# zgojcic/3D_multiview_reg

Measured on AMD Instinct MI355X. Metric: point-cloud pairs/s (feat+match+filter+SVD), 3DMatch 20k-pt, 1/2/4/8 GPU, higher is better.
Workload: dtype f32 (bf16x3 MFMA operands); 1 GPU; one synthetic 3DMatch-scale scene per GPU (configs[2]): 30 fragments x ~20393 voxels (0.025 m) -> FCGF -> rand 5000 samples -> soft feature-NN for all 435 pairs -> OANet (128ch, 500 clusters, 2 blocks) -> weighted Procrustes -> all-gather of (R,t,conf); sampler=rand, fragments_per_gpu=30, pairs_per_gpu=435, samples=5000, voxels_mean=20393, math=f32eq, oanet_point_layout=chunk-major, spconv_presplit_planes=False, spatial_map_order=False, library=353b56b98378a74a, parallelism=dp1 (one scene per rank, RCCL all-gather of records)

## Files before the change

### 3d_multiview_reg_amd/csrc/oan_attn.hip

```cpp
#include <algorithm>
#include <functional>
#include <vector>

#include "common.hpp"
#include "gemm.hpp"
#include "knobs.hpp"
#include "mfma_bf16.hpp"
#include "prof.hpp"
#include "mvreg.h"

namespace mvr {

using namespace bx;

constexpr int AC = 128;
constexpr int AKB = 32;
constexpr int AQ = 256;
constexpr int ATHREADS = 512;
constexpr int ATL = AQ + 4;
constexpr int PLANE = AC * AKB * 2;
constexpr int IMG = 3 * PLANE;
constexpr int STAGE_B = 2 * IMG;
constexpr int MAX_CLUSTERS = 1024;
constexpr int WROW = 272;
constexpr int WPLANE = 32 * WROW;
constexpr int WIMG = 27 * 1024;
constexpr int USTAGE = WIMG + IMG;
static_assert(3 * WPLANE <= WIMG, "W image padding");
constexpr float LOG2E = 1.4426950408889634f;
constexpr float A_NEG = -3.0e38f;
static_assert(64 * ATL * 4 <= 2 * STAGE_B, "epilogue half tile must fit the stage ring");


__device__ int g_attn_reruns;
constexpr float F16_FLOOR = 0.125f;
constexpr float W_SUM_MAX = 128.f;
__device__ __forceinline__ bool v_row_bad(float rmax) { return !(rmax < F16_RANGE) || (rmax > 0.f && rmax < F16_FLOOR); }

#define SCHED_FENCE() __builtin_amdgcn_sched_barrier(0)

#ifndef ATTN_TRACE
#define ATTN_TRACE 0
#endif
#if ATTN_TRACE
__device__ unsigned long long g_attn_trace[16];
#define ATSTAMP(slot)                                                  \
  do {                                                                 \
    unsigned long long t_;                                             \
    __builtin_amdgcn_sched_barrier(0);                                 \
    asm volatile("s_memtime %0\n\ts_waitcnt lgkmcnt(0)" : "=s"(t_));  \
    __builtin_amdgcn_sched_barrier(0);                                 \
    tr_[prev_] += t_ - tlast_;                                         \
    tlast_ = t_;                                                       \
    prev_ = (slot);                                                    \
  } while (0)
#define ATSTART() unsigned long long tr_[8] = {0, 0, 0, 0, 0, 0, 0, 0}, tlast_ = __builtin_amdgcn_s_memtime(); int prev_ = 7
#define ATEND(base)                                                                  \
  do {                                                                               \
    ATSTAMP(7);                                                                      \
    if ((threadIdx.x & 63) == 0)                                                     \
      for (int q_ = 0; q_ < 8; ++q_) atomicAdd(&g_attn_trace[(base) + q_], tr_[q_]); \
  } while (0)
#else
#define ATSTAMP(slot) do {} while (0)
#define ATSTART() do {} while (0)
#define ATEND(base) do {} while (0)
#endif
#define ATTN_INTERLEAVE6()                          \
  do {                                              \
    _Pragma("unroll") for (int u_ = 0; u_ < 6; ++u_) { \
      __builtin_amdgcn_sched_group_barrier(0x008, 1, 0); \
      __builtin_amdgcn_sched_group_barrier(0x002, 5, 0); \
      __builtin_amdgcn_sched_group_barrier(0x200, 1, 0); \
    }                                               \
  } while (0)
#define ATTN_INTERLEAVE3()                          \
  do {                                              \
    _Pragma("unroll") for (int u_ = 0; u_ < 3; ++u_) { \
      __builtin_amdgcn_sched_group_barrier(0x008, 1, 0); \
      __builtin_amdgcn_sched_group_barrier(0x002, 7, 0); \
      __builtin_amdgcn_sched_group_barrier(0x200, 1, 0); \
    }                                               \
  } while (0)

__device__ __forceinline__ int kord_off(int row, int q) {
  const int s = q >> 2, a = (q >> 1) & 1, h = q & 1;
  return row * 64 + 16 * ((2 * s + h) ^ ((row >> 2) & 3)) + 8 * a;
}
__device__ __forceinline__ Frag kord_frag(const char* img, int row, int s, int h) {
  const int off = row * 64 + 16 * ((2 * s + h) ^ ((row >> 2) & 3));
  Frag f;
  f.h = *reinterpret_cast<const bf16x8*>(img + off);
  f.m = *reinterpret_cast<const bf16x8*>(img + PLANE + off);
  f.l = *reinterpret_cast<const bf16x8*>(img + 2 * PLANE + off);
  return f;
}

template <int X>
__device__ __forceinline__ float swz_x(float v) {
  return __int_as_float(__builtin_amdgcn_ds_swizzle(__float_as_int(v), 0x1F | (X << 10)));
}
__device__ __forceinline__ float half_sum(float v) {
  v += swz_x<1>(v);
  v += swz_x<2>(v);
  v += swz_x<4>(v);
  v += swz_x<8>(v);
  v += swz_x<16>(v);
  return v;
}

__device__ __forceinline__ void pair_block(int nblk, int& p, int& blk) {
  const int b = blockIdx.x, x = b & 7, t = b >> 3;
  blk = t % nblk;
  p = (t / nblk) * 8 + x;
}

constexpr float RESCALE = 8.f;
template <int PSH = 0>
__device__ __forceinline__ void online_softmax(float (&v)[16], float& m, float& l, floatx16 (&O)[4]) {
  float bm = __builtin_fmaxf(__builtin_fmaxf(v[0], v[1]), v[2]);
#pragma unroll
  for (int r = 3; r < 15; r += 2) bm = __builtin_fmaxf(__builtin_fmaxf(bm, v[r]), v[r + 1]);
  bm = fmaxf(bm, v[15]);
  bm = fmaxf(bm, __shfl_xor(bm, 32, 64));
  if (__any(bm > m + RESCALE)) {
    const float mn = fmaxf(m, bm);
    const float alpha = __builtin_amdgcn_exp2f(m - mn);
    m = mn;
    l *= alpha;
#pragma unroll
    for (int cb = 0; cb < 4; ++cb) O[cb] *= alpha;
  }
  const float ms = m - (float)PSH;
  float ps = 0.f;
#pragma unroll
  for (int r = 0; r < 16; ++r) {
    v[r] = __builtin_amdgcn_exp2f(v[r] - ms);
    ps += v[r];
  }
  l += ps;
}

__device__ __forceinline__ int64_t cm_off(int n, int64_t cs) { return (int64_t)(n >> 5) * cs + (n & 31); }

__device__ __forceinline__ void tile_out(float* T, const floatx16 (&O)[4], float inv, bool colok, float* out,
                                         int64_t ld, int64_t cs, int col0, int L, float2* st, int64_t st_tile) {
  const int tid = threadIdx.x, lane = tid & 63, w = tid >> 6, l32 = lane & 31, h = lane >> 5;
  const int col = 32 * w + l32;
  const int Lp = (L + 3) & ~3;
  const int nv = min(max(L - col0 - 128 * h, 0), 128);
  const float rnv = nv > 0 ? 1.f / (float)nv : 0.f;
  bool ok[4];
#pragma unroll
  for (int u = 0; u < 4; ++u) ok[u] = 4 * l32 + u < nv;
// ... 444 lines not shown
  const float* sc; const float* sh; int64_t sps;
  const char* wimg;
  const float* bias;
  const float2* bs;
  const char* dimg;
  int P, N, Kc, nkb, nqb;
  float* out; int64_t ops, old, ocs;
  float2* stats; int64_t st_ld; int st_off;
  int* range;
  const int* guard;
};


__global__ __launch_bounds__(ATHREADS) void oan_unpool_kernel(UnpoolArgs a) {
  __shared__ __attribute__((aligned(16))) char smem[USTAGE + 64 * 1024];
  __shared__ __attribute__((aligned(16))) float bsh[MAX_CLUSTERS];
  __shared__ float2 ssh[AC];
  const int tid = threadIdx.x, lane = tid & 63, w = tid >> 6, l32 = lane & 31, h = lane >> 5;
  int p, nb;
  pair_block(a.nqb, p, nb);
  if (p >= a.P) return;
  const int N = a.N, nkb = a.nkb;
  const char* dimg = a.dimg + (int64_t)p * nkb * IMG;

  auto issue = [&](int kb, int st) {
    char* dst = smem + st * USTAGE;
    for (int off = w * 1024; off < USTAGE; off += 8 * 1024) {
      const char* src = off < WIMG ? a.wimg + (int64_t)kb * WIMG + off : dimg + (int64_t)kb * IMG + (off - WIMG);
      glds16b(src + 16 * lane, dst + off);
    }
  };
  issue(0, 0);

  for (int i = tid; i < nkb * AKB; i += ATHREADS)
    bsh[i] = i < a.Kc ? (a.bias ? a.bias[i] * LOG2E : 0.f) : -__builtin_inff();
  if (tid < AC) ssh[tid] = make_float2(a.sc[(int64_t)p * a.sps + tid], a.sh[(int64_t)p * a.sps + tid]);

  const int n = nb * AQ + 32 * w + l32;
  const bool nok = n < N;
  const int nlast = ((N + 3) & ~3) - 4;
  const float* xb = a.X + (int64_t)p * a.xps + cm_off(min(nb * AQ + 4 * lane, nlast), a.xcs);
  auto qdma = [&](int qt) {
    char* dst = smem + USTAGE + (qt & 1) * 32768;
#pragma unroll
    for (int i = 0; i < 4; ++i) {
      const int r = 4 * w + i;
      glds16b(reinterpret_cast<const char*>(xb + (int64_t)(32 * qt + r) * a.xld), dst + r * 1024);
    }
  };
  qdma(0);
  Frag q[8];
#pragma unroll
  for (int qt = 0; qt < 4; ++qt) {
    if (qt < 3) {
      qdma(qt + 1);
      asm volatile("s_waitcnt vmcnt(4)" ::: "memory");
    } else {
      asm volatile("s_waitcnt vmcnt(0)" ::: "memory");
    }
    __syncthreads();
    const float* xt = reinterpret_cast<const float*>(smem + USTAGE + (qt & 1) * 32768) + 32 * w + l32;
#pragma unroll
    for (int kk = 0; kk < 2; ++kk) {
      const int ks = 2 * qt + kk;
      float v[8];
#pragma unroll
      for (int i = 0; i < 8; ++i) {
        const int c = 16 * ks + 8 * h + i;
        const float2 f = ssh[c];
        const float x = fmaxf(fmaf(xt[(c - 32 * qt) * 256], f.x, f.y), 0.f);
        v[i] = nok ? x : 0.f;
      }
      split8(v, q[ks].h, q[ks].m, q[ks].l);
    }
    __syncthreads();
  }

  floatx16 O[4];
#pragma unroll
  for (int cb = 0; cb < 4; ++cb)
#pragma unroll
    for (int r = 0; r < 16; ++r) O[cb][r] = 0.f;
  float m = A_NEG, l = 0.f;

  const int wbase = l32 * WROW + 16 * h;
  auto read_w = [&](const char* Wi, int ks) {
    const int off = wbase + 32 * ks;
    Frag f;
    f.h = *reinterpret_cast<const bf16x8*>(Wi + off);
    f.m = *reinterpret_cast<const bf16x8*>(Wi + WPLANE + off);
    f.l = *reinterpret_cast<const bf16x8*>(Wi + 2 * WPLANE + off);
    return f;
  };

  asm volatile("s_waitcnt vmcnt(0)" ::: "memory");
  __syncthreads();
  for (int kb = 0; kb < nkb; ++kb) {
    const int st = kb & 1;
    if (kb + 1 < nkb) issue(kb + 1, st ^ 1);
    const char* Wi = smem + st * USTAGE;
    const char* D = Wi + WIMG;
    floatx16 S;
#pragma unroll
    for (int r4 = 0; r4 < 4; ++r4) {
      const float4 b = *reinterpret_cast<const float4*>(bsh + kb * AKB + 8 * r4 + 4 * h);
      S[4 * r4 + 0] = b.x;
      S[4 * r4 + 1] = b.y;
      S[4 * r4 + 2] = b.z;
      S[4 * r4 + 3] = b.w;
    }
    Frag cur = read_w(Wi, 0);
#pragma unroll
    for (int ks = 0; ks < 8; ++ks) {
      Frag nxt;
      if (ks < 7) nxt = read_w(Wi, ks + 1);
      SCHED_FENCE();
      S = mfma6(cur, q[ks], S);
      SCHED_FENCE();
      if (ks < 7) cur = nxt;
    }
    Frag df = kord_frag(D, l32, 0, h);
    float v[16];
#pragma unroll
    for (int r = 0; r < 16; ++r) v[r] = S[r];
    online_softmax(v, m, l, O);
    Frag pf[2];
    split8(v, pf[0].h, pf[0].m, pf[0].l);
    split8(v + 8, pf[1].h, pf[1].m, pf[1].l);
#pragma unroll
    for (int i = 0; i < 8; ++i) {
      const int s = i >> 2, cb = i & 3;
      Frag nxt;
      if (i < 7) nxt = kord_frag(D, 32 * ((i + 1) & 3) + l32, (i + 1) >> 2, h);
      SCHED_FENCE();
      O[cb] = mfma6(df, pf[s], O[cb]);
      SCHED_FENCE();
      if (i < 7) df = nxt;
    }
    asm volatile("s_waitcnt vmcnt(0)" ::: "memory");
    __syncthreads();
  }
  const float lt = l + __shfl_xor(l, 32, 64);
  const float inv = lt > 0.f ? 1.f / lt : 0.f;
  const int ntile = (N + 127) / 128;
  tile_out(reinterpret_cast<float*>(smem), O, inv, nok, a.out + (int64_t)p * a.ops, a.old, a.ocs, nb * AQ, N,
           a.stats ? a.stats + ((int64_t)p * ntile + 2 * nb) * a.st_ld + a.st_off : nullptr, a.st_ld);
}

constexpr int U4T = 256;
constexpr int U4Q = 128;
constexpr int U4QB = 32 * U4Q * 4;
constexpr int U4TL = U4Q + 4;
template <int H> constexpr int u4_wimg() { return planes<H>() * WPLANE; }
template <int H> constexpr int u4_lds() { return 2 * u4_wimg<H>() + ximg_bytes<H>(); }
static_assert(u4_wimg<0>() + 2 * U4QB <= u4_lds<0>() && u4_wimg<1>() + 2 * U4QB <= u4_lds<1>(),
              "prologue quarters (at the second W buffer) fit");
static_assert(64 * U4TL * 4 <= u4_lds<1>(), "epilogue half tile fits");

template <int H>
__global__ __launch_bounds__(U4T, 2) void oan_unpool4_kernel(UnpoolArgs a) {
  constexpr int WI4 = u4_wimg<H>();
  constexpr int XDO = 2 * WI4;
  constexpr int XIMG = ximg_bytes<H>();
  constexpr int WSTR = wimg_stride<H>();
  __shared__ __attribute__((aligned(16))) char smem[u4_lds<H>()];
  __shared__ __attribute__((aligned(16))) float bsh[512];
  __shared__ __attribute__((aligned(16))) float ish[H ? 512 : 4];
  __shared__ float2 ssh[AC];
  if (a.guard) {
    if (*a.guard == 0) return;
    if (blockIdx.x == 0 && threadIdx.x == 0) atomicAdd(&g_attn_reruns, 1);
  }
  const int tid = threadIdx.x, lane = tid & 63, w = tid >> 6, l32 = lane & 31, h = lane >> 5;
  int p, nb;
  pair_block(a.nqb, p, nb);
  if (p >= a.P) return;
  ATSTART();
  ATSTAMP(0);
  const int N = a.N, nkb = a.nkb;
  const char* dimg = a.dimg + (int64_t)p * nkb * XIMG;

  const uint32_t smem_lds = lds_addr(smem);
  const int wu = __builtin_amdgcn_readfirstlane(w);
  auto issue_w = [&](int kb) {
    const uint32_t dst = smem_lds + (uint32_t)((kb & 1) * WI4);
    const char* src = a.wimg + (int64_t)kb * WSTR;
#pragma unroll
    for (int i = 0; i < (WI4 + 4095) / 4096; ++i) {
      const int off = wu * 1024 + 4096 * i;
      if (off < WI4 && off + 16 * lane < WI4) glds16s(src, (uint32_t)(off + 16 * lane), dst + (uint32_t)off);
    }
  };
  auto issue_xd = [&](int kb) {
    const char* src = dimg + (int64_t)kb * XIMG;
#pragma unroll
    for (int i = 0; i < (XIMG + 4095) / 4096; ++i) {
      const int off = wu * 1024 + 4096 * i;
      if (off < XIMG) glds16s(src, (uint32_t)(off + 16 * lane), smem_lds + (uint32_t)(XDO + off));
    }
  };
  issue_w(0);

  for (int i = tid; i < nkb * AKB; i += U4T) {
    const float2 b = a.bs[i];
    bsh[i] = b.x;
    if (H) ish[i] = b.y;
  }
  if (tid < AC) ssh[tid] = make_float2(a.sc[(int64_t)p * a.sps + tid], a.sh[(int64_t)p * a.sps + tid]);

  const int n = nb * U4Q + 32 * w + l32;
  const bool nok = n < N;
  const int nlast = ((N + 3) & ~3) - 4;
  const float* xb = a.X + (int64_t)p * a.xps + cm_off(min(nb * U4Q + 4 * l32, nlast), a.xcs);
  auto qdma = [&](int qt) {
    char* dst = smem + WI4 + (qt & 1) * U4QB;
#pragma unroll
    for (int i = 0; i < 4; ++i) {
      const int r2 = 4 * w + i;
      glds16b(reinterpret_cast<const char*>(xb + (int64_t)(32 * qt + 2 * r2 + h) * a.xld), dst + r2 * 1024);
    }
  };
  qdma(0);
  FragT<H> q[8];
  float xmax = 0.f;
#pragma unroll
  for (int qt = 0; qt < 4; ++qt) {
    if (qt < 3) {
      qdma(qt + 1);
      asm volatile("s_waitcnt vmcnt(4)" ::: "memory");
    } else {
      asm volatile("s_waitcnt vmcnt(0)" ::: "memory");
    }
    __syncthreads();
    const float* xt = reinterpret_cast<const float*>(smem + WI4 + (qt & 1) * U4QB) + 32 * w + l32;
#pragma unroll
    for (int kk = 0; kk < 2; ++kk) {
      const int ks = 2 * qt + kk;
      float v[8];
#pragma unroll
      for (int i = 0; i < 8; ++i) {
        const int c = 16 * ks + 8 * h + i;
        const float2 f = ssh[c];
        const float x = fmaxf(fmaf(xt[(c - 32 * qt) * U4Q], f.x, f.y), 0.f);
        v[i] = nok ? x : 0.f;
        if (H) xmax = fmaxf(xmax, v[i]);
      }
      q[ks] = split8t<H>(v);
    }
    __syncthreads();
  }
  if (H && __any(!(xmax < F16_RANGE)) && lane == 0) atomicOr(a.range, 1);
  issue_xd(0);

  floatx16 O[4];
#pragma unroll
  for (int cb = 0; cb < 4; ++cb)
#pragma unroll
    for (int r = 0; r < 16; ++r) O[cb][r] = 0.f;
  float m = A_NEG, l = 0.f;

  const int wbase = l32 * WROW + 16 * h;
  auto read_w = [&](const char* Wi, int ks) { return ld_frag<H>(Wi + wbase + 32 * ks, WPLANE); };
  auto d_frag = [&](const char* D, int row, int s) {
    return ld_frag<H>(D + row * 64 + 16 * ((2 * s + h) ^ ((row >> 2) & 3)), PLANE);
  };

  for (int kb = 0; kb < nkb; ++kb) {
    ATSTAMP(1);
    if (kb + 1 < nkb) issue_w(kb + 1);
    const char* Wi = smem + (kb & 1) * WI4;
    const char* D = smem + XDO;
    floatx16 S;
#pragma unroll
    for (int r4 = 0; r4 < 4; ++r4) {
      const float4 b = *reinterpret_cast<const float4*>(bsh + kb * AKB + 8 * r4 + 4 * h);
      S[4 * r4 + 0] = b.x;
      S[4 * r4 + 1] = b.y;
      S[4 * r4 + 2] = b.z;
      S[4 * r4 + 3] = b.w;
    }
    FragT<H> cur = read_w(Wi, 0);
#pragma unroll
    for (int ks = 0; ks < 8; ++ks) {
      FragT<H> nxt;
      if (ks < 7) nxt = read_w(Wi, ks + 1);
      SCHED_FENCE();
      S = mma<H>(cur, q[ks], S);
      SCHED_FENCE();
      if (ks < 7) cur = nxt;
    }
    ATSTAMP(2);
    float v[16];
    if (H) {
#pragma unroll
      for (int r4 = 0; r4 < 4; ++r4) {
        const float4 is = *reinterpret_cast<const float4*>(ish + kb * AKB + 8 * r4 + 4 * h);
        v[4 * r4 + 0] = S[4 * r4 + 0] * is.x;
        v[4 * r4 + 1] = S[4 * r4 + 1] * is.y;
        v[4 * r4 + 2] = S[4 * r4 + 2] * is.z;
        v[4 * r4 + 3] = S[4 * r4 + 3] * is.w;
      }
    } else {
#pragma unroll
      for (int r = 0; r < 16; ++r) v[r] = S[r];
    }
    online_softmax<H ? 7 : 0>(v, m, l, O);
    FragT<H> pf[2] = {split8t<H>(v), split8t<H>(v + 8)};
    ATSTAMP(3);
    asm volatile("s_waitcnt vmcnt(0)" ::: "memory");
    __syncthreads();
    ATSTAMP(4);
    FragT<H> df = d_frag(D, l32, 0);
#pragma unroll
    for (int i = 0; i < 8; ++i) {
      const int s = i >> 2, cb = i & 3;
      FragT<H> nxt;
      if (i < 7) nxt = d_frag(D, 32 * ((i + 1) & 3) + l32, (i + 1) >> 2);
      SCHED_FENCE();
      O[cb] = mma<H>(df, pf[s], O[cb]);
      SCHED_FENCE();
      if (i < 7) df = nxt;
    }
    ATSTAMP(5);
    __syncthreads();
    if (kb + 1 < nkb) issue_xd(kb + 1);
  }
  asm volatile("s_waitcnt vmcnt(0)" ::: "memory");
  __syncthreads();
  ATSTAMP(6);

  const float lt = l + __shfl_xor(l, 32, 64);
  const float inv = lt > 0.f ? 1.f / lt : 0.f;
  float* T = reinterpret_cast<float*>(smem);
  const int col0 = nb * U4Q;
  const int nv = min(max(N - col0, 0), U4Q);
  const float rnv = nv > 0 ? 1.f / (float)nv : 0.f;
  bool ok[4];
#pragma unroll
  for (int u = 0; u < 4; ++u) ok[u] = 4 * l32 + u < nv;
  const int Lp = (N + 3) & ~3;
  const bool sok = col0 + 4 * l32 < Lp;
  float* out = a.out + (int64_t)p * a.ops;
  float2* st = a.stats ? a.stats + ((int64_t)p * ((N + 127) / 128) + nb) * a.st_ld + a.st_off : nullptr;
#pragma unroll
  for (int hf = 0; hf < 2; ++hf) {
#pragma unroll
    for (int cc = 0; cc < 2; ++cc)
#pragma unroll
      for (int q2 = 0; q2 < 16; ++q2) {
        const int c = 32 * cc + (q2 & 3) + 8 * (q2 >> 2) + 4 * h;
        T[c * U4TL + 32 * w + l32] = nok ? O[2 * hf + cc][q2] * inv : 0.f;
      }
    __syncthreads();
    for (int it = 0; it < 8; ++it) {
      const int cl = 16 * w + 2 * it + h, c = 64 * hf + cl;
      float4 x = *reinterpret_cast<const float4*>(T + cl * U4TL + 4 * l32);
      if (!ok[0]) x.x = 0.f;
      if (!ok[1]) x.y = 0.f;
      if (!ok[2]) x.z = 0.f;
      if (!ok[3]) x.w = 0.f;
      if (st) {
        const float sm = half_sum((x.x + x.y) + (x.z + x.w));
        const float mu = sm * rnv;
        const float d0 = ok[0] ? x.x - mu : 0.f, d1 = ok[1] ? x.y - mu : 0.f, d2 = ok[2] ? x.z - mu : 0.f,
                    d3 = ok[3] ? x.w - mu : 0.f;
        const float m2 = half_sum((d0 * d0 + d1 * d1) + (d2 * d2 + d3 * d3));
        if (l32 == 0 && nv > 0) st[c] = make_float2(sm, m2);
      }
      if (sok) *reinterpret_cast<float4*>(out + (int64_t)c * a.old + cm_off(col0 + 4 * l32, a.ocs)) = x;
    }
    __syncthreads();
  }
  ATEND(8);
}

#ifndef ATTN_MATH_DEFAULT
#define ATTN_MATH_DEFAULT 0
#endif
int g_attn_h = ATTN_MATH_DEFAULT;

}

using namespace mvr;

static bool al16(const void* p) { return (reinterpret_cast<uintptr_t>(p) & 15) == 0; }
static int64_t round_up4(int64_t x) { return (x + 3) & ~(int64_t)3; }

#if ATTN_TRACE
extern "C" int mvr_attn_trace(unsigned long long* out, int reset) {
  if (hipMemcpyFromSymbol(out, HIP_SYMBOL(mvr::g_attn_trace), sizeof(unsigned long long) * 16) != hipSuccess) return -1;
  if (reset) {
    unsigned long long z[16] = {};
    if (hipMemcpyToSymbol(HIP_SYMBOL(mvr::g_attn_trace), z, sizeof(z)) != hipSuccess) return -1;
  }
  return 0;
}
#endif

extern "C" size_t mvr_oan_diff_unpool_workspace_bytes(int P, int channels, int clusters) {
  if (P <= 0 || channels != AC || clusters <= 0 || clusters > MAX_CLUSTERS) return 0;
  const size_t nkb = (size_t)(clusters + AKB - 1) / AKB;
  return nkb * (WIMG + (size_t)P * IMG + AKB * sizeof(float2)) + 512;
}

struct PoolSplit { int nks, g0; };
#ifndef POOL_TAIL
#define POOL_TAIL 0
#endif
static double pool_makespan(int64_t full, int64_t parts, int k, int cus) {
  std::vector<double> slot((size_t)cus, 0.0);
  std::make_heap(slot.begin(), slot.end(), std::greater<double>());
  auto put = [&](double d) {
    std::pop_heap(slot.begin(), slot.end(), std::greater<double>());
    slot.back() += d;
    std::push_heap(slot.begin(), slot.end(), std::greater<double>());
  };
  for (int64_t i = 0; i < full; ++i) put(1.0);
  for (int64_t i = 0; i < parts; ++i) put(1.0 / k);
  return *std::max_element(slot.begin(), slot.end());
}
static PoolSplit pool_splits(int P, int nqb, int N) {
  const int nkb = (N + AKB - 1) / AKB;
  if (!POOL_TAIL) return nkb >= 16 ? PoolSplit{2, 0} : PoolSplit{1, (P + 7) / 8};
  int dev = 0, cus = 0;
  if (hipGetDevice(&dev) != hipSuccess ||
      hipDeviceGetAttribute(&cus, hipDeviceAttributeMultiprocessorCount, dev) != hipSuccess || cus <= 0)
    cus = 256;
  const int G = (P + 7) / 8;
  const int64_t per = 8LL * nqb;
  PoolSplit best{1, G};
  double tbest = pool_makespan(per * G, 0, 1, cus);
  int64_t slabs_best = 0;
  for (int k = 2; k <= 4; k *= 2) {
    if (nkb < 8 * k) break;
    const int gfill = (int)(((per * G) / cus) * cus / per);
    const int cands[3] = {0, gfill, G};
    for (int g0 : cands) {
      if (g0 >= G) continue;
      const int64_t parts = per * k * (G - g0);
      const double t = pool_makespan(per * g0, parts, k, cus);
      if (t < tbest - 1e-9 || (t < tbest + 1e-9 && parts < slabs_best)) {
        tbest = t;
        best = PoolSplit{k, g0};
        slabs_best = parts;
      }
    }
  }
  return best;
}

static size_t pool_ws_bytes(int P, int clusters, int nks) {
  const size_t slots = (size_t)P * ((clusters + AQ - 1) / AQ);
  return (nks > 1 ? slots * ((size_t)nks * PSLAB * 4 + 4) : 0) + 512;
}


extern "C" size_t mvr_oan_diff_pool_workspace_bytes(int P, int channels, int clusters) {
  if (P <= 0 || channels != AC || clusters <= 0 || clusters > MAX_CLUSTERS) return 0;
  return pool_ws_bytes(P, clusters, 4);
}

extern "C" int mvr_oan_diff_pool_ws(const float* x, int64_t x_pstride, int64_t x_ld, const float* sc,
                                    const float* sh, int64_t s_pstride, const float* weight, const float* bias, int P,
                                    int channels, int N, int clusters, float* out, int64_t out_pstride, int64_t out_ld,
                                    float* stats, int64_t st_ld, int st_off, void* workspace, size_t workspace_bytes,
                                    hipStream_t stream);

extern "C" int mvr_oan_diff_pool(const float* x, int64_t x_pstride, int64_t x_ld, const float* sc, const float* sh,
                                 int64_t s_pstride, const float* weight, const float* bias, int P, int channels, int N,
                                 int clusters, float* out, int64_t out_pstride, int64_t out_ld, float* stats,
                                 int64_t st_ld, int st_off, hipStream_t stream) {
  return mvr_oan_diff_pool_ws(x, x_pstride, x_ld, sc, sh, s_pstride, weight, bias, P, channels, N, clusters, out,
                              out_pstride, out_ld, stats, st_ld, st_off, nullptr, 0, stream);
}

extern "C" int mvr_oan_diff_pool_ws(const float* x, int64_t x_pstride, int64_t x_ld, const float* sc,
                                    const float* sh, int64_t s_pstride, const float* weight, const float* bias, int P,
                                    int channels, int N, int clusters, float* out, int64_t out_pstride, int64_t out_ld,
                                    float* stats, int64_t st_ld, int st_off, void* workspace, size_t workspace_bytes,
                                    hipStream_t stream) {
  return mvr::oan_diff_pool_cm(x, x_pstride, x_ld, 32, sc, sh, s_pstride, weight, bias, P, channels, N, clusters, out,
                               out_pstride, out_ld, stats, st_ld, st_off, workspace, workspace_bytes, stream);
}

int mvr::oan_diff_pool_cm(const float* x, int64_t x_pstride, int64_t x_ld, int64_t x_cs, const float* sc,
                          const float* sh, int64_t s_pstride, const float* weight, const float* bias, int P,
                          int channels, int N, int clusters, float* out, int64_t out_pstride, int64_t out_ld,
                          float* stats, int64_t st_ld, int st_off, void* workspace, size_t workspace_bytes,
                          hipStream_t stream) {
  if (P < 0 || N <= 0 || channels != AC || clusters <= 0 || clusters > MAX_CLUSTERS) return MVR_EINVAL;
  if (P == 0) return MVR_OK;
  if (!x || !sc || !sh || !weight || !out) return MVR_EINVAL;
  const bool xcm = x_cs != 32;
  if ((xcm ? (x_ld != 32 || (x_cs & 3) || x_cs < 32 * AC) : x_ld < round_up4(N)) || (x_ld & 3) || (x_pstride & 3) ||
      !al16(x) || !al16(weight) || !al16(out) || out_ld < round_up4(clusters) || (out_ld & 3) || (out_pstride & 3) ||
      (stats && (st_ld < channels + st_off)))
    return MVR_EINVAL;
  if ((xcm ? (int64_t)((N + 31) / 32) * x_cs : (int64_t)AC * x_ld) * 4 >= ((int64_t)1 << 31)) return MVR_EINVAL;
  if (P == 0) return MVR_OK;
  PoolArgs a{};
  a.X = x; a.xps = x_pstride; a.xld = x_ld; a.xcs = x_cs;
  a.sc = sc; a.sh = sh; a.sps = s_pstride;
  a.W = weight; a.bias = bias;
  a.P = P; a.N = N; a.Kc = clusters; a.nqb = (clusters + AQ - 1) / AQ;
  a.out = out; a.ops = out_pstride; a.old = out_ld;
  a.stats = reinterpret_cast<float2*>(stats); a.st_ld = st_ld; a.st_off = st_off;
  a.nks = 1;
  const size_t slots = (size_t)P * a.nqb;
  int* range = nullptr;
  if (workspace) {
    if (!al16(workspace) || workspace_bytes < pool_ws_bytes(P, clusters, 4)) return MVR_EINVAL;
    const PoolSplit ps = pool_splits(P, a.nqb, N);
    const int k = ps.nks;
    if (k > 1) {
      a.nks = k;
      a.g0 = ps.g0;
      a.part = reinterpret_cast<float*>(workspace);
      a.cnt = reinterpret_cast<int*>(reinterpret_cast<char*>(workspace) + slots * (size_t)k * PSLAB * 4);
    }
    if (g_attn_h)
      range = reinterpret_cast<int*>(reinterpret_cast<char*>(workspace) +
                                     (a.nks > 1 ? slots * ((size_t)a.nks * PSLAB * 4 + 4) : 0));
  }
  if (a.nks > 1 || range) {
    void* z = a.nks > 1 ? (void*)a.cnt : (void*)range;
// ... 116 lines not shown
```

Baseline: 11090 pairs/s.

## Software-pipeline unpool attention: overlap softmax/split with next block's MFMA

Restructures the OANet unpool attention kernel so that the softmax and bf16/f16 operand split for key block j run interleaved with the score MFMAs of block j+1. It also interleaves the output MFMAs, using sched_group_barrier hints and per-plane fragment reloads. The LDS layout changes from a double-buffered W image to a single W image plus double-buffered x_down images, and the prologue gets a deeper ring of X quarter loads. Waves whose columns are entirely out of range now skip the math. The goal is to hide VALU softmax latency behind MFMA and cut serialization, at the cost of more complex scheduling, extra register pressure and a different barrier pattern.

```diff
diff --git a/3d_multiview_reg_amd/csrc/oan_attn.hip b/3d_multiview_reg_amd/csrc/oan_attn.hip
--- a/3d_multiview_reg_amd/csrc/oan_attn.hip
+++ b/3d_multiview_reg_amd/csrc/oan_attn.hip
@@ -1,5 +1,6 @@
 #include <algorithm>
 #include <functional>
+#include <type_traits>
 #include <vector>
 
 #include "common.hpp"
@@ -750,15 +751,62 @@
 constexpr int U4QB = 32 * U4Q * 4;
 constexpr int U4TL = U4Q + 4;
 template <int H> constexpr int u4_wimg() { return planes<H>() * WPLANE; }
-template <int H> constexpr int u4_lds() { return 2 * u4_wimg<H>() + ximg_bytes<H>(); }
+template <int H> constexpr int u4_lds() { return u4_wimg<H>() + 2 * ximg_bytes<H>(); }
 static_assert(u4_wimg<0>() + 2 * U4QB <= u4_lds<0>() && u4_wimg<1>() + 2 * U4QB <= u4_lds<1>(),
-              "prologue quarters (at the second W buffer) fit");
+              "prologue quarters (behind the W image, over the x_down slots) fit");
 static_assert(64 * U4TL * 4 <= u4_lds<1>(), "epilogue half tile fits");
+static_assert(u4_lds<0>() <= 76800, "two workgroups per CU");
+
+template <typename V16>
+__device__ __forceinline__ void softmax_decide(const V16& v, float& m, float& l, float& alpha, bool& resc) {
+  float bm = __builtin_fmaxf(__builtin_fmaxf(v[0], v[1]), v[2]);
+#pragma unroll
+  for (int r = 3; r < 15; r += 2) bm = __builtin_fmaxf(__builtin_fmaxf(bm, v[r]), v[r + 1]);
+  bm = fmaxf(bm, v[15]);
+  bm = fmaxf(bm, __shfl_xor(bm, 32, 64));
+  resc = __any(bm > m + RESCALE);
+  const float mn = fmaxf(m, bm);
+  alpha = __builtin_amdgcn_exp2f(m - mn);
+  l = resc ? l * alpha : l;
+  m = resc ? mn : m;
+}
+template <int H, typename LD>
+__device__ __forceinline__ floatx16 mma_reload(FragT<H>& a, const FragT<H>& b, floatx16 acc, LD ld) {
+  if constexpr (H) {
+    acc = __builtin_amdgcn_mfma_f32_32x32x16_f16(a.p[1], b.p[0], acc, 0, 0, 0);
+    a.p[1] = ld(1);
+    acc = __builtin_amdgcn_mfma_f32_32x32x16_f16(a.p[0], b.p[1], acc, 0, 0, 0);
+    acc = __builtin_amdgcn_mfma_f32_32x32x16_f16(a.p[0], b.p[0], acc, 0, 0, 0);
+  } else {
+    acc = __builtin_amdgcn_mfma_f32_32x32x16_bf16(a.p[2], b.p[0], acc, 0, 0, 0);
+    a.p[2] = ld(2);
+    acc = __builtin_amdgcn_mfma_f32_32x32x16_bf16(a.p[0], b.p[2], acc, 0, 0, 0);
+    acc = __builtin_amdgcn_mfma_f32_32x32x16_bf16(a.p[1], b.p[1], acc, 0, 0, 0);
+    acc = __builtin_amdgcn_mfma_f32_32x32x16_bf16(a.p[1], b.p[0], acc, 0, 0, 0);
+    a.p[1] = ld(1);
+    acc = __builtin_amdgcn_mfma_f32_32x32x16_bf16(a.p[0], b.p[1], acc, 0, 0, 0);
+    acc = __builtin_amdgcn_mfma_f32_32x32x16_bf16(a.p[0], b.p[0], acc, 0, 0, 0);
+  }
+  return acc;
+}
+#define ATTN_MIX_LD(NV)                                   \
+  do {                                                    \
+    __builtin_amdgcn_sched_group_barrier(0x008, 1, 0);    \
+    __builtin_amdgcn_sched_group_barrier(0x100, 1, 0);    \
+    __builtin_amdgcn_sched_group_barrier(0x002, (NV), 0); \
+  } while (0)
+#define ATTN_MIX(NM, NV)                                    \
+  do {                                                      \
+    _Pragma("unroll") for (int u_ = 0; u_ < (NM); ++u_) {   \
+      __builtin_amdgcn_sched_group_barrier(0x008, 1, 0);    \
+      __builtin_amdgcn_sched_group_barrier(0x002, (NV), 0); \
+    }                                                       \
+  } while (0)
 
 template <int H>
 __global__ __launch_bounds__(U4T, 2) void oan_unpool4_kernel(UnpoolArgs a) {
   constexpr int WI4 = u4_wimg<H>();
-  constexpr int XDO = 2 * WI4;
+  constexpr int XDO = WI4;
   constexpr int XIMG = ximg_bytes<H>();
   constexpr int WSTR = wimg_stride<H>();
   __shared__ __attribute__((aligned(16))) char smem[u4_lds<H>()];
@@ -780,57 +828,62 @@
 
   const uint32_t smem_lds = lds_addr(smem);
   const int wu = __builtin_amdgcn_readfirstlane(w);
+  uint32_t voff = (uint32_t)(wu * 1024 + 16 * lane);
+  asm volatile("" : "+v"(voff));
   auto issue_w = [&](int kb) {
-    const uint32_t dst = smem_lds + (uint32_t)((kb & 1) * WI4);
     const char* src = a.wimg + (int64_t)kb * WSTR;
 #pragma unroll
     for (int i = 0; i < (WI4 + 4095) / 4096; ++i) {
       const int off = wu * 1024 + 4096 * i;
-      if (off < WI4 && off + 16 * lane < WI4) glds16s(src, (uint32_t)(off + 16 * lane), dst + (uint32_t)off);
+      const bool whole = 4096 * (i + 1) <= WI4;
+      if (whole || (off < WI4 && off + 16 * lane < WI4)) glds16s(src + 4096 * i, voff, smem_lds + (uint32_t)off);
     }
   };
   auto issue_xd = [&](int kb) {
     const char* src = dimg + (int64_t)kb * XIMG;
-#pragma unroll
-    for (int i = 0; i < (XIMG + 4095) / 4096; ++i) {
+    static_assert(XIMG % 4096 == 0, "whole rounds of 4 x 1 KB");
+#pragma unroll
+    for (int i = 0; i < XIMG / 4096; ++i) {
       const int off = wu * 1024 + 4096 * i;
-      if (off < XIMG) glds16s(src, (uint32_t)(off + 16 * lane), smem_lds + (uint32_t)(XDO + off));
+      glds16s(src + 4096 * i, voff, smem_lds + (uint32_t)(XDO + (kb & 1) * XIMG + off));
     }
   };
   issue_w(0);
 
-  for (int i = tid; i < nkb * AKB; i += U4T) {
-    const float2 b = a.bs[i];
-    bsh[i] = b.x;
-    if (H) ish[i] = b.y;
-  }
-  if (tid < AC) ssh[tid] = make_float2(a.sc[(int64_t)p * a.sps + tid], a.sh[(int64_t)p * a.sps + tid]);
-
+  constexpr int NQB = H ? 2 : 3;
+  static_assert(WI4 + NQB * U4QB <= u4_lds<H>(), "prologue ring");
   const int n = nb * U4Q + 32 * w + l32;
   const bool nok = n < N;
   const int nlast = ((N + 3) & ~3) - 4;
   const float* xb = a.X + (int64_t)p * a.xps + cm_off(min(nb * U4Q + 4 * l32, nlast), a.xcs);
   auto qdma = [&](int qt) {
-    char* dst = smem + WI4 + (qt & 1) * U4QB;
+    char* dst = smem + WI4 + (qt % NQB) * U4QB;
 #pragma unroll
     for (int i = 0; i < 4; ++i) {
       const int r2 = 4 * w + i;
       glds16b(reinterpret_cast<const char*>(xb + (int64_t)(32 * qt + 2 * r2 + h) * a.xld), dst + r2 * 1024);
     }
   };
-  qdma(0);
+#pragma unroll
+  for (int qt = 0; qt < NQB; ++qt) qdma(qt);
+
+  for (int i = tid; i < nkb * AKB; i += U4T) {
+    const float2 b = a.bs[i];
+    bsh[i] = b.x;
+    if (H) ish[i] = b.y;
+  }
+  if (tid < AC) ssh[tid] = make_float2(a.sc[(int64_t)p * a.sps + tid], a.sh[(int64_t)p * a.sps + tid]);
+
   FragT<H> q[8];
   float xmax = 0.f;
 #pragma unroll
   for (int qt = 0; qt < 4; ++qt) {
-    if (qt < 3) {
-      qdma(qt + 1);
-      asm volatile("s_waitcnt vmcnt(4)" ::: "memory");
-    } else {
-      asm volatile("s_waitcnt vmcnt(0)" ::: "memory");
-    }
+    const int newer = NQB - 1 < 3 - qt ? NQB - 1 : 3 - qt;
+    if (newer == 2) asm volatile("s_waitcnt vmcnt(8)" ::: "memory");
+    else if (newer == 1) asm volatile("s_waitcnt vmcnt(4)" ::: "memory");
+    else asm volatile("s_waitcnt vmcnt(0)" ::: "memory");
     __syncthreads();
-    const float* xt = reinterpret_cast<const float*>(smem + WI4 + (qt & 1) * U4QB) + 32 * w + l32;
+    const float* xt = reinterpret_cast<const float*>(smem + WI4 + (qt % NQB) * U4QB) + 32 * w + l32;
 #pragma unroll
     for (int kk = 0; kk < 2; ++kk) {
       const int ks = 2 * qt + kk;
@@ -846,6 +899,7 @@
       q[ks] = split8t<H>(v);
     }
     __syncthreads();
+    if (qt + NQB < 4) qdma(qt + NQB);
   }
   if (H && __any(!(xmax < F16_RANGE)) && lane == 0) atomicOr(a.range, 1);
   issue_xd(0);
@@ -863,112 +917,219 @@
     return ld_frag<H>(D + row * 64 + 16 * ((2 * s + h) ^ ((row >> 2) & 3)), PLANE);
   };
 
-  for (int kb = 0; kb < nkb; ++kb) {
-    ATSTAMP(1);
-    if (kb + 1 < nkb) issue_w(kb + 1);
-    const char* Wi = smem + (kb & 1) * WI4;
-    const char* D = smem + XDO;
-    floatx16 S;
+  const bool wact = nb * U4Q + 32 * wu < N;
+  floatx16 S;
+  float v[16];
+  FragT<H> pf[2];
+  typedef std::true_type Yes;
+  typedef std::false_type No;
+
+  auto phase1 = [&](int j, auto split) {
+    constexpr bool SPLIT = decltype(split)::value;
+    const char* Wi = smem;
 #pragma unroll
     for (int r4 = 0; r4 < 4; ++r4) {
-      const float4 b = *reinterpret_cast<const float4*>(bsh + kb * AKB + 8 * r4 + 4 * h);
+      const float4 b = *reinterpret_cast<const float4*>(bsh + j * AKB + 8 * r4 + 4 * h);
       S[4 * r4 + 0] = b.x;
       S[4 * r4 + 1] = b.y;
       S[4 * r4 + 2] = b.z;
       S[4 * r4 + 3] = b.w;
     }
+    unsigned pt[8][3];
     FragT<H> cur = read_w(Wi, 0);
 #pragma unroll
     for (int ks = 0; ks < 8; ++ks) {
-      FragT<H> nxt;
-      if (ks < 7) nxt = read_w(Wi, ks + 1);
+      auto w_plane = [&](int pl) {
+        return *reinterpret_cast<const typename FragT<H>::V*>(Wi + wbase + 32 * (ks + 1) + pl * WPLANE);
+      };
+      typename FragT<H>::V nx0;
+      if (ks < 7) nx0 = w_plane(0);
       SCHED_FENCE();
-      S = mma<H>(cur, q[ks], S);
+      if (SPLIT) {
+        asm volatile("" : "+v"(v[2 * ks]), "+v"(v[2 * ks + 1]));
+        split_pair<H>(f32x2{v[2 * ks], v[2 * ks + 1]}, pt[ks]);
+      }
+      if (ks < 7) {
+        S = mma_reload<H>(cur, q[ks], S, w_plane);
+        if (SPLIT && H) {
+          ATTN_MIX_LD(4);
+          ATTN_MIX(2, 4);
+        } else if (SPLIT) {
+          ATTN_MIX_LD(2);
+          ATTN_MIX(2, 2);
+          ATTN_MIX_LD(2);
+          ATTN_MIX(2, 2);
+        }
+      } else {
+        S = mma<H>(cur, q[ks], S);
+        if (SPLIT) {
+          if (H) ATTN_MIX(3, 4); else ATTN_MIX(6, 2);
+        }
+      }
+      if (SPLIT) {
+        if (H) asm volatile("" ::"v"(pt[ks][0]), "v"(pt[ks][1]));
+        else asm volatile("" ::"v"(pt[ks][0]), "v"(pt[ks][1]), "v"(pt[ks][2]));
+      }
       SCHED_FENCE();
-      if (ks < 7) cur = nxt;
-    }
+      if (ks < 7) cur.p[0] = nx0;
+    }
+    if (SPLIT) {
+#pragma unroll
+      for (int s = 0; s < 2; ++s)
+#pragma unroll
+        for (int pl = 0; pl < planes<H>(); ++pl)
+          pf[s].p[pl] = __builtin_bit_cast(typename FragT<H>::V, u32x4{pt[4 * s][pl], pt[4 * s + 1][pl],
+                                                                       pt[4 * s + 2][pl], pt[4 * s + 3][pl]});
+    }
+  };
+  auto phase2 = [&](int j, auto soft, auto mm) {
+    constexpr bool SOFT = decltype(soft)::value, MM = decltype(mm)::value;
+    constexpr int R0[9] = {0, 0, 3, 6, 8, 10, 12, 14, 16};
+    const char* D = smem + XDO + ((j - 1) & 1) * XIMG;
+    float alpha = 1.f, ms = 0.f, ps = 0.f;
+    bool resc = false;
+    FragT<H> df;
+    if (MM) df = d_frag(D, l32, 0);
+#pragma unroll
+    for (int i = 0; i < 8; ++i) {
+      const int s = i >> 2, cb = i & 3;
+      const char* Dn = D + (32 * ((i + 1) & 3) + l32) * 64 + 16 * ((2 * ((i + 1) >> 2) + h) ^ ((l32 >> 2) & 3));
+      auto d_plane = [&](int pl) { return *reinterpret_cast<const typename FragT<H>::V*>(Dn + pl * PLANE); };
+      typename FragT<H>::V nx0;
+      if (MM && i < 7) nx0 = d_plane(0);
+      SCHED_FENCE();
+      if (SOFT) {
+        if (i == 0) {
+          if (H) {
+#pragma unroll
+            for (int r4 = 0; r4 < 4; ++r4) {
+              const float4 is = *reinterpret_cast<const float4*>(ish + j * AKB + 8 * r4 + 4 * h);
+              S[4 * r4 + 0] *= is.x;
+              S[4 * r4 + 1] *= is.y;
+              S[4 * r4 + 2] *= is.z;
+              S[4 * r4 + 3] *= is.w;
+            }
+          }
+          softmax_decide(S, m, l, alpha, resc);
+          ms = m - (float)(H ? 7 : 0);
+        } else {
+          asm volatile("" : "+v"(ms));
+        }
+#pragma unroll
+        for (int r = R0[i]; r < R0[i + 1]; ++r) {
+          v[r] = __builtin_amdgcn_exp2f(S[r] - ms);
+          ps += v[r];
+        }
+        if (i == 7) l += ps;
+      }
+      if (MM && i < 7) {
+        O[cb] = mma_reload<H>(df, pf[s], O[cb], d_plane);
+        if (SOFT && H) {
+          ATTN_MIX_LD(4);
+          ATTN_MIX(2, 4);
+        } else if (SOFT) {
+          ATTN_MIX_LD(2);
+          ATTN_MIX(2, 2);
+          ATTN_MIX_LD(2);
+          ATTN_MIX(2, 2);
+        }
+      } else if (MM) {
+        O[cb] = mma<H>(df, pf[s], O[cb]);
+        if (SOFT) {
+          if (H) ATTN_MIX(3, 4); else ATTN_MIX(6, 2);
+        }
+      }
+      if (SOFT) asm volatile("" ::"v"(ps), "v"(l));
+      SCHED_FENCE();
+      if (MM && i < 7) df.p[0] = nx0;
+    }
+    if (SOFT && resc) {
+#pragma unroll
+      for (int cb = 0; cb < 4; ++cb) O[cb] *= alpha;
+    }
+  };
+
+  ATSTAMP(1);
+  if (wact) phase1(0, No());
+  ATSTAMP(2);
+  __syncthreads();
+  if (nkb > 1) issue_w(1);
+  ATSTAMP(3);
+  if (wact) phase2(0, Yes(), No());
+  ATSTAMP(4);
+  asm volatile("s_waitcnt vmcnt(0)" ::: "memory");
+  __syncthreads();
+  if (nkb > 1) issue_xd(1);
+  for (int j = 1; j < nkb; ++j) {
+    ATSTAMP(1);
+    if (wact) phase1(j, Yes());
     ATSTAMP(2);
-    float v[16];
-    if (H) {
-#pragma unroll
-      for (int r4 = 0; r4 < 4; ++r4) {
-        const float4 is = *reinterpret_cast<const float4*>(ish + kb * AKB + 8 * r4 + 4 * h);
-        v[4 * r4 + 0] = S[4 * r4 + 0] * is.x;
-        v[4 * r4 + 1] = S[4 * r4 + 1] * is.y;
-        v[4 * r4 + 2] = S[4 * r4 + 2] * is.z;
-        v[4 * r4 + 3] = S[4 * r4 + 3] * is.w;
-      }
-    } else {
-#pragma unroll
-      for (int r = 0; r < 16; ++r) v[r] = S[r];
-    }
-    online_softmax<H ? 7 : 0>(v, m, l, O);
-    FragT<H> pf[2] = {split8t<H>(v), split8t<H>(v + 8)};
+    __syncthreads();
+    if (j + 1 < nkb) issue_w(j + 1);
     ATSTAMP(3);
+    if (wact) phase2(j, Yes(), Yes());
+    ATSTAMP(4);
     asm volatile("s_waitcnt vmcnt(0)" ::: "memory");
     __syncthreads();
-    ATSTAMP(4);
-    FragT<H> df = d_frag(D, l32, 0);
-#pragma unroll
-    for (int i = 0; i < 8; ++i) {
-      const int s = i >> 2, cb = i & 3;
-      FragT<H> nxt;
-      if (i < 7) nxt = d_frag(D, 32 * ((i + 1) & 3) + l32, (i + 1) >> 2);
-      SCHED_FENCE();
-      O[cb] = mma<H>(df, pf[s], O[cb]);
-      SCHED_FENCE();
-      if (i < 7) df = nxt;
-    }
-    ATSTAMP(5);
-    __syncthreads();
-    if (kb + 1 < nkb) issue_xd(kb + 1);
-  }
-  asm volatile("s_waitcnt vmcnt(0)" ::: "memory");
+    if (j + 1 < nkb) issue_xd(j + 1);
+  }
+  ATSTAMP(5);
+  if (wact) {
+    pf[0] = split8t<H>(v);
+    pf[1] = split8t<H>(v + 8);
+    phase2(nkb, No(), Yes());
+  }
   __syncthreads();
   ATSTAMP(6);
 
-  const float lt = l + __shfl_xor(l, 32, 64);
-  const float inv = lt > 0.f ? 1.f / lt : 0.f;
-  float* T = reinterpret_cast<float*>(smem);
-  const int col0 = nb * U4Q;
-  const int nv = min(max(N - col0, 0), U4Q);
-  const float rnv = nv > 0 ? 1.f / (float)nv : 0.f;
-  bool ok[4];
-#pragma unroll
-  for (int u = 0; u < 4; ++u) ok[u] = 4 * l32 + u < nv;
-  const int Lp = (N + 3) & ~3;
-  const bool sok = col0 + 4 * l32 < Lp;
-  float* out = a.out + (int64_t)p * a.ops;
-  float2* st = a.stats ? a.stats + ((int64_t)p * ((N + 127) / 128) + nb) * a.st_ld + a.st_off : nullptr;
-#pragma unroll
-  for (int hf = 0; hf < 2; ++hf) {
-#pragma unroll
-    for (int cc = 0; cc < 2; ++cc)
-#pragma unroll
-      for (int q2 = 0; q2 < 16; ++q2) {
-        const int c = 32 * cc + (q2 & 3) + 8 * (q2 >> 2) + 4 * h;
-        T[c * U4TL + 32 * w + l32] = nok ? O[2 * hf + cc][q2] * inv : 0.f;
-      }
-    __syncthreads();
-    for (int it = 0; it < 8; ++it) {
-      const int cl = 16 * w + 2 * it + h, c = 64 * hf + cl;
-      float4 x = *reinterpret_cast<const float4*>(T + cl * U4TL + 4 * l32);
-      if (!ok[0]) x.x = 0.f;
-      if (!ok[1]) x.y = 0.f;
-      if (!ok[2]) x.z = 0.f;
-      if (!ok[3]) x.w = 0.f;
-      if (st) {
-        const float sm = half_sum((x.x + x.y) + (x.z + x.w));
-        const float mu = sm * rnv;
-        const float d0 = ok[0] ? x.x - mu : 0.f, d1 = ok[1] ? x.y - mu : 0.f, d2 = ok[2] ? x.z - mu : 0.f,
-                    d3 = ok[3] ? x.w - mu : 0.f;
-        const float m2 = half_sum((d0 * d0 + d1 * d1) + (d2 * d2 + d3 * d3));
-        if (l32 == 0 && nv > 0) st[c] = make_float2(sm, m2);
-      }
-      if (sok) *reinterpret_cast<float4*>(out + (int64_t)c * a.old + cm_off(col0 + 4 * l32, a.ocs)) = x;
-    }
-    __syncthreads();
-  }
+  int te = tid;
+  asm volatile("" : "+v"(te));
+  [&](const int lane, const int w) {
+    const int l32 = lane & 31, h = lane >> 5;
+    const bool nok = nb * U4Q + 32 * w + l32 < N;
+    const float lt = l + __shfl_xor(l, 32, 64);
+    const float inv = lt > 0.f ? 1.f / lt : 0.f;
+    float* T = reinterpret_cast<float*>(smem);
+    const int col0 = nb * U4Q;
+    const int nv = min(max(N - col0, 0), U4Q);
+    const float rnv = nv > 0 ? 1.f / (float)nv : 0.f;
+    bool ok[4];
+#pragma unroll
+    for (int u = 0; u < 4; ++u) ok[u] = 4 * l32 + u < nv;
+    const int Lp = (N + 3) & ~3;
+    const bool sok = col0 + 4 * l32 < Lp;
+    float* out = a.out + (int64_t)p * a.ops;
+    float2* st = a.stats ? a.stats + ((int64_t)p * ((N + 127) / 128) + nb) * a.st_ld + a.st_off : nullptr;
+#pragma unroll
+    for (int hf = 0; hf < 2; ++hf) {
+#pragma unroll
+      for (int cc = 0; cc < 2; ++cc)
+#pragma unroll
+        for (int q2 = 0; q2 < 16; ++q2) {
+          const int c = 32 * cc + (q2 & 3) + 8 * (q2 >> 2) + 4 * h;
+          T[c * U4TL + 32 * w + l32] = nok ? O[2 * hf + cc][q2] * inv : 0.f;
+        }
+      __syncthreads();
+      for (int it = 0; it < 8; ++it) {
+        const int cl = 16 * w + 2 * it + h, c = 64 * hf + cl;
+        float4 x = *reinterpret_cast<const float4*>(T + cl * U4TL + 4 * l32);
+        if (!ok[0]) x.x = 0.f;
+        if (!ok[1]) x.y = 0.f;
+        if (!ok[2]) x.z = 0.f;
+        if (!ok[3]) x.w = 0.f;
+        if (st) {
+          const float sm = half_sum((x.x + x.y) + (x.z + x.w));
+          const float mu = sm * rnv;
+          const float d0 = ok[0] ? x.x - mu : 0.f, d1 = ok[1] ? x.y - mu : 0.f, d2 = ok[2] ? x.z - mu : 0.f,
+                      d3 = ok[3] ? x.w - mu : 0.f;
+          const float m2 = half_sum((d0 * d0 + d1 * d1) + (d2 * d2 + d3 * d3));
+          if (l32 == 0 && nv > 0) st[c] = make_float2(sm, m2);
+        }
+        if (sok) *reinterpret_cast<float4*>(out + (int64_t)c * a.old + cm_off(col0 + 4 * l32, a.ocs)) = x;
+      }
+      __syncthreads();
+    }
+  }(te & 63, te >> 6);
   ATEND(8);
 }
 
```

New measurement: 11160 pairs/s (median of 6 runs). No clear change (+0.6%).
